# al-mcintyre/mCaller

Measured on NVIDIA B200. Metric: per-read site calls/sec, higher is better.
Workload: dtype f64

## Files before the change

### include/mcaller_b200.h

```cpp
#ifndef MCALLER_B200_H
#define MCALLER_B200_H

#include <stdint.h>

#ifdef __cplusplus
extern "C" {
#endif

#define MC_ABI_VERSION 3

#define MC_TILE_BYTES 3840
#define MC_TEXT_PAD 4096
#define MC_MAXK 8

enum {
    MC_OK = 0,
    MC_EINVAL = -1,
    MC_ECUDA = -2,
    MC_ECAPACITY = -3
};

typedef struct mc_refindex {
    int32_t n_contigs;
    int32_t k;
// ... 15 lines not shown
    uint16_t line_hi;
    uint16_t name_off;
    int32_t pos;
    int32_t event_idx;
    double diff;
    uint16_t name_len;
    uint16_t contig;
    uint8_t flags;
    uint8_t kbits_fwd;
    uint8_t kbits_rev;
    uint8_t pad;
} mc_record;

#define MC_RF_EQ 1u
#define MC_RF_CAND 2u
#define MC_RF_BADNUM 4u
#define MC_RF_BADIDX 8u
#define MC_RF_RAW 16u
#define MC_RF_NEWREAD 32u
#define MC_RF_SEGKNOWN 64u

enum {
    MC_C_LINES = 0,
    MC_C_KEPT,
    MC_C_RECORDS,
    MC_C_SHORT,
    MC_C_UNKNOWN_CONTIG,
    MC_C_NNN,
    MC_C_BADPOS,
    MC_C_LONGLINE,
    MC_C_OVERFLOW,
    MC_C_RUN_CURSOR,
    MC_C_QUIET,
    MC_C_COUNT = 16
};

typedef struct mc_call {
    int64_t read_off;
    double prob;
    double feat[MC_MAXK + 1];
    int32_t read_len;
    int32_t mpos;
    int32_t site;
    uint32_t close_rec;
    uint16_t win_contig;
    uint16_t chrom_contig;
    uint8_t kind;
    uint8_t rev;
    uint8_t n_empty;
    uint8_t empty_mask;
    uint8_t model_sel;
    uint8_t label;
    uint8_t err;
    uint8_t pad0;
    uint32_t seg;
    uint32_t pad1;
    uint32_t pad2;
} mc_call;

enum { MC_CALL = 0, MC_TOO_MANY_SKIPS = 1, MC_MULTI_M = 2, MC_NONE = 3  };
#define MC_CE_CONTEXT 1u
#define MC_CE_MODELKEY 2u
#define MC_CE_BADNUM 4u
#define MC_CE_COLUMN 8u
#define MC_CE_SPACING 16u

// ... 9 lines not shown
    const double *d_biases;
    int32_t n_trees;
    int32_t max_nodes;
    const int32_t *d_tree_off;
    const int32_t *d_left;
    const int32_t *d_right;
    const int32_t *d_feature;
    const double *d_threshold;
    const double *d_leaf_p1;
} mc_model;

typedef struct mc_qual_entry {
    uint64_t hash;
    uint32_t check;
    uint32_t len;
    double qual;
} mc_qual_entry;


int mc_version(void);
int mc_sizeof(int what);
const char *mc_last_error(void);

int mc_read_u64(const uint64_t *d_src, int64_t n, uint64_t *h_dst, void *stream);

int mc_scan(const uint8_t *d_text, int64_t nbytes, const mc_refindex *ref, int dense,
            mc_record *d_rec, int64_t rec_cap, uint32_t *d_tile_tab , uint32_t *d_run_tab ,
            uint64_t *d_counters, void *stream);

int mc_scan_run_len(int64_t nbytes);

int mc_scan_set_run_len(int run_len);

int64_t mc_num_tiles(int64_t nbytes);

int64_t mc_workspace_bytes(int64_t n);

int mc_order_records(const uint8_t *d_text, int64_t nbytes, const mc_refindex *ref, const uint32_t *d_tile_tab, int64_t n_tiles,
                     uint32_t *d_run_tab, int run_len, const mc_record *d_rec_in, int64_t rec_in_cap, const uint64_t *d_scan_counters,
                     mc_record *d_rec_out, int64_t rec_out_cap, uint64_t *d_n_out, uint32_t *d_seg_flags ,
                     uint32_t *d_run_first , void *d_ws, void *stream);

int mc_segment_reads(const uint8_t *d_text, mc_record *d_rec, const uint64_t *d_n_records, int64_t rec_cap,
                     uint32_t *d_seg_flags , const uint32_t *d_run_first, int64_t n_runs,
                     uint32_t *d_seg_start, uint64_t *d_nseg, void *d_ws, void *stream);

int mc_segment_quality(const uint8_t *d_text, const mc_record *d_rec, const uint32_t *d_seg_start, const uint64_t *d_nseg,
                       int64_t seg_cap, const mc_qual_entry *d_table, int64_t table_size, double *d_seg_qual, uint64_t *d_err,
                       void *stream);

int mc_build_windows(const mc_record *d_rec, const uint64_t *d_n_records, int64_t rec_cap, const uint32_t *d_seg_start,
                     const uint64_t *d_nseg, int64_t seg_cap, const double *d_seg_qual, const mc_refindex *ref, int skip_thresh,
                     double qual_thresh, int two_models, mc_call *d_calls, int64_t call_cap, uint32_t *d_seg_count,
                     uint64_t *d_ncalls, void *d_ws, double *d_spill, int64_t spill_cap, void *stream);

typedef struct mc_carry {
    mc_call row;
    uint32_t valid;
    int32_t first_kept_contig;
    uint64_t chunks;
    uint64_t pad[6];
} mc_carry;
int mc_carry_reset(mc_carry *d_carry, void *stream);
int mc_carry_rows(mc_call *d_rows, const uint64_t *d_ncalls, const mc_record *d_rec, const uint64_t *d_n_records,
                  const uint32_t *d_seg_start, const uint64_t *d_nseg, const double *d_seg_qual, double qual_thresh,
                  mc_carry *d_carry, uint64_t *d_nrows_out, const uint64_t *d_abort, void *stream);
// ... 103 lines not shown
```

### mcaller_b200/_lib.py

```python
import ctypes as C
import os

import numpy as np

HERE = os.path.dirname(os.path.abspath(__file__))
LIB_PATH = os.environ.get("MCALLER_B200_LIB") or os.path.join(HERE, "libmcaller_b200.so")

MC_TILE_BYTES = 3840
MC_TEXT_PAD = 4096
MC_MAXK = 8
MC_C_COUNT = 16
COUNTER_NAMES = ["lines", "kept", "records", "short", "unknown_contig", "nnn", "badpos", "longline", "overflow", "run_cursor", "quiet_chunks"]

MC_ABI_VERSION = 3
MC_CALL, MC_TOO_MANY_SKIPS, MC_MULTI_M, MC_NONE = 0, 1, 2, 3
MC_CE_CONTEXT, MC_CE_MODELKEY, MC_CE_BADNUM, MC_CE_COLUMN, MC_CE_SPACING = 1, 2, 4, 8, 16
MC_MLP, MC_LR, MC_GNB, MC_RF = 0, 1, 2, 3
PENDING = 0xFFFFFFFF


class RefIndex(C.Structure):
    _fields_ = [("n_contigs", C.c_int32), ("k", C.c_int32), ("d_names", C.c_void_p), ("d_name_off", C.c_void_p),
                ("d_base", C.c_void_p), ("d_len", C.c_void_p), ("d_site_fwd", C.c_void_p), ("d_site_rev", C.c_void_p),
                ("d_cand", C.c_void_p), ("d_rank_fwd", C.c_void_p), ("d_rank_rev", C.c_void_p), ("d_bases", C.c_void_p),
                ("total_bits", C.c_int64)]


class Model(C.Structure):
    _fields_ = [("kind", C.c_int32), ("n_in", C.c_int32), ("n_layers", C.c_int32), ("hidden_act", C.c_int32),
                ("sizes", C.c_int32 * 8), ("d_weights", C.c_void_p), ("d_biases", C.c_void_p), ("n_trees", C.c_int32),
                ("max_nodes", C.c_int32), ("d_tree_off", C.c_void_p), ("d_left", C.c_void_p), ("d_right", C.c_void_p),
                ("d_feature", C.c_void_p), ("d_threshold", C.c_void_p), ("d_leaf_p1", C.c_void_p)]


class SynthSpec(C.Structure):
    _fields_ = [("seed", C.c_uint64), ("n_contigs", C.c_int32), ("len_min", C.c_int32), ("len_max", C.c_int32),
                ("p_skip", C.c_int32), ("p_nnn", C.c_int32), ("margin", C.c_int32), ("meth", C.c_int32),
                ("d_names", C.c_void_p), ("d_name_off", C.c_void_p), ("d_contig_len", C.c_void_p),
                ("d_read_bounds", C.c_void_p), ("d_gbase", C.c_void_p), ("d_genome", C.c_void_p),
                ("d_meth_fwd", C.c_void_p), ("d_meth_rev", C.c_void_p), ("d_model_mean", C.c_void_p),
                ("d_model_sd", C.c_void_p)]


RECORD_DTYPE = np.dtype([("line_lo", "<u4"), ("line_hi", "<u2"), ("name_off", "<u2"), ("pos", "<i4"), ("event_idx", "<i4"),
                         ("diff", "<f8"), ("name_len", "<u2"), ("contig", "<u2"), ("flags", "u1"), ("kbits_fwd", "u1"), ("kbits_rev", "u1"), ("pad", "u1")])
# ... 12 lines not shown
class TrainJob(C.Structure):
    _fields_ = [("d_x", C.c_void_p), ("d_y", C.c_void_p), ("d_w", C.c_void_p), ("d_loss_curve", C.c_void_p), ("idx_off", C.c_int64),
                ("n", C.c_int32), ("d", C.c_int32), ("max_iter", C.c_int32), ("n_iter_no_change", C.c_int32), ("alpha", C.c_double),
                ("lr", C.c_double), ("tol", C.c_double), ("best_loss", C.c_double), ("n_iter", C.c_int32), ("no_improve", C.c_int32),
                ("stopped", C.c_int32), ("pad", C.c_int32)]


MC_TRAIN_HIDDEN, MC_TRAIN_BATCH = 100, 200

CARRY_BYTES = 192

QUAL_DTYPE = np.dtype([("hash", "<u8"), ("check", "<u4"), ("len", "<u4"), ("qual", "<f8")])
assert QUAL_DTYPE.itemsize == 24
DIFFS_ROW_DTYPE = np.dtype([("line_off", "<u8"), ("slot", "<u4"), ("values_off", "<u4"), ("values_len", "<u4"), ("prob_off", "<u4"),
                            ("prob_len", "<u4"), ("pad", "<u4")])
assert DIFFS_ROW_DTYPE.itemsize == 32


class McallerCudaError(RuntimeError):
    pass


_lib = None

_PROTOS = {
    "mc_version": (C.c_int, []),
    "mc_sizeof": (C.c_int, [C.c_int]),
    "mc_last_error": (C.c_char_p, []),
    "mc_read_u64": (C.c_int, [C.c_void_p, C.c_int64, C.c_void_p, C.c_void_p]),
    "mc_scan": (C.c_int, [C.c_void_p, C.c_int64, C.POINTER(RefIndex), C.c_int, C.c_void_p, C.c_int64, C.c_void_p, C.c_void_p, C.c_void_p,
                          C.c_void_p]),
    "mc_scan_run_len": (C.c_int, [C.c_int64]),
    "mc_scan_set_run_len": (C.c_int, [C.c_int]),
    "mc_num_tiles": (C.c_int64, [C.c_int64]),
    "mc_workspace_bytes": (C.c_int64, [C.c_int64]),
    "mc_order_records": (C.c_int, [C.c_void_p, C.c_int64, C.POINTER(RefIndex), C.c_void_p, C.c_int64, C.c_void_p, C.c_int, C.c_void_p,
                                   C.c_int64, C.c_void_p, C.c_void_p, C.c_int64, C.c_void_p, C.c_void_p, C.c_void_p, C.c_void_p, C.c_void_p]),
    "mc_segment_reads": (C.c_int, [C.c_void_p, C.c_void_p, C.c_void_p, C.c_int64, C.c_void_p, C.c_void_p, C.c_int64, C.c_void_p, C.c_void_p,
                                   C.c_void_p, C.c_void_p]),
    "mc_segment_quality": (C.c_int, [C.c_void_p, C.c_void_p, C.c_void_p, C.c_void_p, C.c_int64, C.c_void_p, C.c_int64, C.c_void_p,
                                     C.c_void_p, C.c_void_p]),
    "mc_build_windows": (C.c_int, [C.c_void_p, C.c_void_p, C.c_int64, C.c_void_p, C.c_void_p, C.c_int64, C.c_void_p, C.POINTER(RefIndex),
                                   C.c_int, C.c_double, C.c_int, C.c_void_p, C.c_int64, C.c_void_p, C.c_void_p, C.c_void_p, C.c_void_p,
                                   C.c_int64, C.c_void_p]),
    "mc_carry_reset": (C.c_int, [C.c_void_p, C.c_void_p]),
    "mc_carry_rows": (C.c_int, [C.c_void_p, C.c_void_p, C.c_void_p, C.c_void_p, C.c_void_p, C.c_void_p, C.c_void_p, C.c_double, C.c_void_p,
                                C.c_void_p, C.c_void_p, C.c_void_p]),
    "mc_chunk_guard": (C.c_int, [C.c_void_p, C.c_int64, C.c_void_p, C.c_int64, C.c_void_p, C.c_int64, C.c_void_p, C.c_int64, C.c_void_p,
                                 C.c_void_p, C.c_void_p]),
    "mc_carry_close": (C.c_int, [C.c_void_p, C.c_int, C.c_void_p, C.c_int, C.c_int, C.c_void_p, C.c_void_p, C.c_void_p, C.c_void_p,
                                 C.c_int64, C.c_void_p, C.c_void_p]),
    "mc_classify_workspace_bytes": (C.c_int64, [C.c_int64]),
    "mc_classify": (C.c_int, [C.c_void_p, C.c_void_p, C.c_int64, C.POINTER(Model), C.c_void_p, C.c_void_p]),
    "mc_hist_accumulate": (C.c_int, [C.c_void_p, C.c_void_p, C.c_int64, C.c_void_p, C.c_void_p, C.c_void_p, C.c_int64, C.c_void_p,
                                     C.c_void_p, C.c_int64, C.c_void_p, C.c_void_p, C.c_void_p]),
    "mc_count_calls": (C.c_int, [C.c_void_p, C.c_void_p, C.c_int64, C.c_void_p, C.c_void_p]),
    "mc_bed_select": (C.c_int, [C.c_void_p, C.c_void_p, C.c_int64, C.c_int64, C.c_double, C.c_int, C.c_void_p, C.c_void_p, C.c_void_p]),
    "mc_format_rows": (C.c_int64, [C.c_void_p, C.c_int64, C.c_void_p, C.c_void_p, C.c_int32, C.c_void_p, C.c_void_p, C.c_void_p, C.c_void_p,
                                   C.c_int32, C.c_int32, C.c_char_p, C.c_char_p, C.c_int32, C.c_int32, C.c_void_p, C.c_int64]),
    "mc_fastq_tiles": (C.c_int64, [C.c_int64]),
    "mc_fastq_index": (C.c_int, [C.c_void_p, C.c_int64, C.c_void_p, C.c_void_p, C.c_void_p, C.c_int64, C.c_void_p, C.c_void_p, C.c_void_p]),
    "mc_fastq_quality": (C.c_int, [C.c_void_p, C.c_int64, C.c_void_p, C.c_int64, C.c_void_p, C.c_int64, C.c_void_p, C.c_void_p, C.c_void_p,
                                   C.c_void_p]),
    "mc_synth_genome": (C.c_int, [C.POINTER(SynthSpec), C.c_void_p, C.c_int64, C.c_void_p]),
    "mc_synth_sizes": (C.c_int, [C.POINTER(SynthSpec), C.c_int64, C.c_int64, C.c_int64, C.c_void_p, C.c_void_p]),
    "mc_synth_write": (C.c_int, [C.POINTER(SynthSpec), C.c_int64, C.c_int64, C.c_int64, C.c_void_p, C.c_void_p, C.c_void_p]),
# ... 37 lines not shown
```

### mcaller_b200/csrc/scan.cu

```cuda
#include "parse.cuh"

namespace {

constexpr int CHUNK = MC_TILE_BYTES;
constexpr int LOOKB = 32;
constexpr int LOOKA = 224;
constexpr int WB = LOOKB + CHUNK + LOOKA;
constexpr int NW = WB / 32;
#ifndef MC_SCAN_WARPS
#define MC_SCAN_WARPS 24
#endif
#ifndef MC_SCAN_MIN_CTAS
#define MC_SCAN_MIN_CTAS 1
#endif
#ifndef MC_SCAN_RUN
#define MC_SCAN_RUN 128
#endif

constexpr int WARPS = MC_SCAN_WARPS;
constexpr int THREADS = WARPS * 32;
constexpr int LCAP = 32;
constexpr int RESERVE = 256;
static_assert(WB == 4096 && NW == 128, "chunk geometry");
static_assert(CHUNK % 16 == 0, "chunks must keep 16-byte alignment");
static_assert(MC_TEXT_PAD >= LOOKA + 64, "text padding must cover the look-ahead");

struct WarpSmem {
    alignas(16) uint8_t text[2][WB];
    alignas(16) uint32_t fs[NW + 8];
    alignas(16) uint32_t nl[NW + 4];
    uint16_t lstart[LCAP + 4];
    uint32_t cnt[8];
    unsigned long long key[4];
    alignas(8) unsigned long long bar[2];
    unsigned long long rname[8];
};

__device__ __forceinline__ uint32_t smem_u32(const void *p) { return (uint32_t)__cvta_generic_to_shared(p); }
__device__ __forceinline__ void mbar_init(unsigned long long *bar, uint32_t count) {
    asm volatile("mbarrier.init.shared::cta.b64 [%0], %1;" ::"r"(smem_u32(bar)), "r"(count) : "memory");
}
__device__ __forceinline__ void fence_barrier_init() { asm volatile("fence.mbarrier_init.release.cluster;" ::: "memory"); }
__device__ __forceinline__ void fence_proxy_async() { asm volatile("fence.proxy.async.shared::cta;" ::: "memory"); }
__device__ __forceinline__ void tma_load_1d(void *dst, const void *src, uint32_t bytes, unsigned long long *bar) {
    asm volatile("mbarrier.arrive.expect_tx.shared::cta.b64 _, [%0], %1;" ::"r"(smem_u32(bar)), "r"(bytes) : "memory");
    asm volatile("cp.async.bulk.shared::cluster.global.mbarrier::complete_tx::bytes [%0], [%1], %2, [%3];" ::"r"(smem_u32(dst)),
                 "l"(src), "r"(bytes), "r"(smem_u32(bar))
                 : "memory");
}
__device__ __forceinline__ bool mbar_wait(unsigned long long *bar, uint32_t parity) {
    const uint32_t a = smem_u32(bar);
    for (uint32_t spin = 0; spin < (1u << 26); ++spin) {
        uint32_t done;
        asm volatile(
            "{\n\t.reg .pred p;\n\t"
            "mbarrier.try_wait.parity.shared::cta.b64 p, [%1], %2;\n\t"
            "selp.u32 %0, 1, 0, p;\n\t}"
            : "=r"(done)
            : "r"(a), "r"(parity)
            : "memory");
        if (done) return true;
    }
    return false;
}

__device__ __forceinline__ uint32_t pack32(uint32_t m0, uint32_t m1, uint32_t m2, uint32_t m3, uint32_t m4, uint32_t m5,
                                           uint32_t m6, uint32_t m7) {
    const uint32_t lo = 0x08040201u, hi = 0x80402010u;
    const uint32_t a = __dp4a(m1, hi, __dp4a(m0, lo, 0u));
    const uint32_t b = __dp4a(m3, hi, __dp4a(m2, lo, 0u));
    const uint32_t c = __dp4a(m5, hi, __dp4a(m4, lo, 0u));
    const uint32_t d = __dp4a(m7, hi, __dp4a(m6, lo, 0u));
    return (a >> 7) + b * 2u + c * 512u + d * 131072u;
}

__device__ __noinline__ int select_fs_walk(const uint32_t *fs, int s, int n) {
    int w = s >> 5;
    uint32_t m = fs[w] & (0xFFFFFFFFu << (s & 31));
    int c = __popc(m);
    while (c <= n) {
        n -= c;
        if (++w >= NW) return NW * 32;
        m = fs[w];
        c = __popc(m);
    }
    for (; n > 0; --n) m &= m - 1u;
    return (w << 5) + __ffs(m) - 1;
}
__device__ __forceinline__ int next_bit(const uint32_t *m, int q) {
    int w = q >> 5;
    uint32_t v = m[w] & (0xFFFFFFFFu << (q & 31));
    while (v == 0u) {
        if (++w >= NW) return NW * 32;
        v = m[w];
    }
    return (w << 5) + __ffs(v) - 1;
}

template <bool WANT3>
__device__ __forceinline__ void line_fields(const WarpSmem &S, int s, int &f0, int &f1, int &f9, int &f11, int &f3) {
    const int w0 = s >> 5, sh = s & 31;
    const uint32_t a0 = S.fs[w0], a1 = S.fs[w0 + 1], a2 = S.fs[w0 + 2], a3 = S.fs[w0 + 3], a4 = S.fs[w0 + 4], a5 = S.fs[w0 + 5];
    const uint32_t W0 = __funnelshift_r(a0, a1, sh), W1 = __funnelshift_r(a1, a2, sh), W2 = __funnelshift_r(a2, a3, sh),
                   W3 = __funnelshift_r(a3, a4, sh), W4 = __funnelshift_r(a4, a5, sh);
    const int c0 = __popc(W0), c1 = c0 + __popc(W1), c2 = c1 + __popc(W2), c3 = c2 + __popc(W3), c4 = c3 + __popc(W4);
    if (c4 >= 12) {
        auto sel = [&](int k) {
            const int wi = (k >= c0) + (k >= c1) + (k >= c2) + (k >= c3);
            const uint32_t m = wi == 0 ? W0 : wi == 1 ? W1 : wi == 2 ? W2 : wi == 3 ? W3 : W4;
            const int base = wi == 0 ? 0 : wi == 1 ? c0 : wi == 2 ? c1 : wi == 3 ? c2 : c3;
            return s + 32 * wi + nth_bit(m, k - base);
        };
        if ((W0 & 1u) && c0 >= 2) {
            f0 = s;
            f1 = s + __ffs(W0 & (W0 - 1u)) - 1;
        } else {
            f0 = sel(0);
            f1 = sel(1);
        }
        if (WANT3) f3 = c0 >= 4 ? s + nth_bit(W0, 3) : sel(3);
        if (c2 <= 9 && c3 > 11) {
            uint32_t m = W3;
            const int j = 9 - c2;
#pragma unroll
            for (int t = 0; t < 4; ++t)
                if (j > t) m &= m - 1u;
            for (int t = 4; t < j; ++t) m &= m - 1u;
            f9 = s + 96 + __ffs(m) - 1;
            m &= m - 1u;
            m &= m - 1u;
            f11 = s + 96 + __ffs(m) - 1;
        } else {
            f9 = sel(9);
            f11 = sel(11);
        }
    } else {
        f0 = select_fs_walk(S.fs, s, 0);
        f1 = select_fs_walk(S.fs, s, 1);
        f9 = select_fs_walk(S.fs, s, 9);
        f11 = select_fs_walk(S.fs, s, 11);
        if (WANT3) f3 = select_fs_walk(S.fs, s, 3);
    }
}

__device__ __forceinline__ unsigned long long load8(const uint8_t *text, int q) {
    const uint32_t *wp = reinterpret_cast<const uint32_t *>(text + (q & ~3));
    const uint32_t w0 = wp[0], w1 = wp[1], w2 = wp[2];
    const int sh = 8 * (q & 3);
    const uint32_t lo = __funnelshift_r(w0, w1, sh), hi = __funnelshift_r(w1, w2, sh);
    return ((unsigned long long)hi << 32) | lo;
}

__device__ __forceinline__ int parse_pos8(unsigned long long k8, int &pos) {
    const uint32_t lo = (uint32_t)k8, hi = (uint32_t)(k8 >> 32);
    const uint32_t xl = lo ^ 0x30303030u, xh = hi ^ 0x30303030u;
    const uint32_t ndl = (((xl & 0x7f7f7f7fu) + 0x76767676u) | lo) & 0x80808080u;
    const uint32_t ndh = (((xh & 0x7f7f7f7fu) + 0x76767676u) | hi) & 0x80808080u;
    if ((ndl | ndh) == 0u) return -1;
    const int n = ndl ? ((__ffs(ndl) - 1) >> 3) : 4 + ((__ffs(ndh) - 1) >> 3);
    const uint32_t term = (n < 4 ? (lo >> (8 * n)) : (hi >> (8 * n - 32))) & 0xFFu;
    if (n == 0 || term > 0x20u) return 0;
    const int sh = 64 - 8 * n;
    const uint32_t H = sh < 32 ? __funnelshift_l(xl, xh, sh) : (xl << (sh - 32));
    const uint32_t L = sh < 32 ? (xl << sh) : 0u;
    pos = (int)(conv4(L) * 10000u + conv4(H));
    return 1;
}

__device__ __forceinline__ int token_len64(const uint8_t *text, int q) {
    for (int j = 0; j < 9; ++j) {
        const unsigned long long v = load8(text, q + 8 * j);
        const uint32_t lo = gt20_msb((uint32_t)v) ^ 0x80808080u, hi = gt20_msb((uint32_t)(v >> 32)) ^ 0x80808080u;
        if (lo) return 8 * j + ((__ffs(lo) - 1) >> 3);
        if (hi) return 8 * j + 4 + ((__ffs(hi) - 1) >> 3);
    }
    return -1;
}
__device__ __forceinline__ unsigned long long low_bytes(unsigned long long v, int n) {
    return n >= 8 ? v : (v & ((1ull << (8 * n)) - 1ull));
}
__device__ __forceinline__ bool token_is(const uint8_t *text, int q, int len, const unsigned long long *key) {
    bool eq = true;
    for (int j = 0; 8 * j < len; ++j) eq = eq && low_bytes(load8(text, q + 8 * j), len - 8 * j) == key[j];
    return eq;
}
__device__ __forceinline__ bool spans_equal(const uint8_t *text, int qa, int qb, int len) {
    bool eq = true;
    for (int j = 0; 8 * j < len; ++j) eq = eq && low_bytes(load8(text, qa + 8 * j) ^ load8(text, qb + 8 * j), len - 8 * j) == 0ull;
    return eq;
}
__device__ __forceinline__ int pos_digits8(unsigned long long k8) {
    const uint32_t lo = (uint32_t)k8, hi = (uint32_t)(k8 >> 32);
    const uint32_t xl = lo ^ 0x30303030u, xh = hi ^ 0x30303030u;
    const uint32_t ndl = (((xl & 0x7f7f7f7fu) + 0x76767676u) | lo) & 0x80808080u;
    const uint32_t ndh = (((xh & 0x7f7f7f7fu) + 0x76767676u) | hi) & 0x80808080u;
    return ndl ? ((__ffs(ndl) - 1) >> 3) : 4 + ((__ffs(ndh) - 1) >> 3);
}

enum { ST_KEPT = 1u, ST_CAND = 2u, ST_SHORT = 4u, ST_UNKNOWN = 8u, ST_NNN = 16u, ST_BADPOS = 32u };
// ... 5 lines not shown
    cid = known_cid >= 0 ? known_cid : contig_lookup(t, f0, R, hint);
    if (cid < 0) return ST_UNKNOWN;
    if (nnn_state > 0 || (nnn_state < 0 && is_nnnnnn(t, f9))) return ST_NNN;
    if (pos_state == 0 || (pos_state < 0 && !parse_uint(t, f1, pos))) return ST_BADPOS;
    uint32_t st = ST_KEPT;
    const int len = (cid == hint) ? hint_len : __ldg(R.d_len + cid);
    if (pos < len) {
        const int64_t g = ((cid == hint) ? hint_base : __ldg(R.d_base + cid)) + pos;
        if ((__ldg(R.d_cand + (g >> 5)) >> (g & 31)) & 1u) st |= ST_CAND;
    }
    return st;
}

__device__ __noinline__ uint32_t classify_from_global(const uint8_t *d_text, int64_t limit, int64_t goff, const mc_refindex &R, int hint,
                                                      int64_t hint_base, int hint_len, int &cid, int &pos) {
    const GlobalBytes t{d_text + goff, limit - goff};
    int nf = 0, f0 = 0, f1 = 0, f9 = 0;
    bool in_tok = false;
    for (int i = 0; i < (1 << 20); ++i) {
        const int c = t[i];
        if (c == 0x0a) break;
        const bool ws = c <= 0x20;
        if (!ws && !in_tok) {
            if (nf == 0) f0 = i; else if (nf == 1) f1 = i; else if (nf == 9) f9 = i;
            ++nf;
            in_tok = true;
            if (nf >= 12) break;
        } else if (ws) in_tok = false;
    }
    if (nf < 12) return ST_SHORT;
    return classify_line(t, f0, f1, f9, R, hint, hint_base, hint_len, -1, -1, -1, cid, pos);
}

template <bool RF>
__global__ void __launch_bounds__(THREADS, MC_SCAN_MIN_CTAS)
k_scan(const uint8_t *__restrict__ d_text, int64_t nbytes, int64_t text_limit16, int64_t n_chunks64, int run_len, mc_refindex R,
       int dense, mc_record *__restrict__ d_rec, unsigned long long rec_cap, uint32_t *__restrict__ d_tile_tab,
       uint32_t *__restrict__ d_run_tab, unsigned long long *__restrict__ d_counters) {
    extern __shared__ __align__(16) uint8_t smem_raw[];
    const int lane = threadIdx.x & 31, wib = threadIdx.x >> 5;
    WarpSmem &S = reinterpret_cast<WarpSmem *>(smem_raw)[wib];
    const int warp_global = (int)blockIdx.x * WARPS + wib;
    const int n_warps = (int)gridDim.x * WARPS;
    const int n_chunks = (int)n_chunks64;
    const int n_runs = (n_chunks + run_len - 1) / run_len;
    const uint32_t lt_mask = (1u << lane) - 1u;

    const uint32_t K7F = 0x7f7f7f7fu | ((uint32_t)((unsigned long long)nbytes >> 63) << 7);
    auto eq0a_r = [&](uint32_t w) -> uint32_t {
        const uint32_t t = ((w ^ 0x0a0a0a0au) & K7F) + K7F;
        return ~(t | w) & 0x80808080u;
    };

    int hint = -1;
    int64_t hint_base = 0;
    int hint_len = 0, hint_nlen = 0;
    unsigned long long hint_key = 0ull;
    auto set_hint = [&](int c) {
        hint = c;
        hint_base = __ldg(R.d_base + c);
        hint_len = __ldg(R.d_len + c);
        const int o0 = __ldg(R.d_name_off + c);
        hint_nlen = __ldg(R.d_name_off + c + 1) - o0;
        hint_key = 0ull;
        for (int j = 0; j < hint_nlen && j < 7; ++j) hint_key |= (unsigned long long)__ldg(R.d_names + o0 + j) << (8 * j);
        __syncwarp();
        if (lane < 4) {
            unsigned long long kk = 0ull;
            for (int j = 8 * lane; j < hint_nlen && j < 8 * lane + 8; ++j) kk |= (unsigned long long)__ldg(R.d_names + o0 + j) << (8 * (j & 7));
            S.key[lane] = kk;
        }
        __syncwarp();
    };
    set_hint(0);
    unsigned long long slot_cur = 0ull;
    unsigned slot_left = 0u;
    unsigned c_lines = 0, c_kept = 0;
    if (lane < 8) S.cnt[lane] = 0u;

    if (lane == 0) {
        mbar_init(&S.bar[0], 1);
        mbar_init(&S.bar[1], 1);
        fence_barrier_init();
    }
    __syncwarp();
    uint32_t phase0 = 0u, phase1 = 0u;

    const int64_t q_hi = text_limit16 - WB + LOOKB, q_tail = nbytes - WB + LOOKB;
    const int c_bulk_hi = q_hi < 0 ? -1 : (int)min(q_hi / CHUNK, (int64_t)0x7fffffff);
    const int c_tail_lo = q_tail < 0 ? 0 : (int)min(q_tail / CHUNK + 1, (int64_t)0x7fffffff);
    auto stage = [&](int c, int b) -> bool {
        const int64_t g0 = (int64_t)c * CHUNK - LOOKB;
        if (c >= 1 && c <= c_bulk_hi) {
            if (lane == 0) {
                fence_proxy_async();
                tma_load_1d(S.text[b], d_text + g0, WB, &S.bar[b]);
            }
            return true;
        }
        for (int i = lane; i < WB / 16; i += 32) {
            const int64_t g = g0 + 16 * i;
            uint4 v = make_uint4(0x0a0a0a0au, 0x0a0a0a0au, 0x0a0a0a0au, 0x0a0a0a0au);
            if (g >= 0 && g < text_limit16) v = __ldg(reinterpret_cast<const uint4 *>(d_text + g));
            *reinterpret_cast<uint4 *>(S.text[b] + 16 * i) = v;
        }
        return false;
    };

    int rname_len = -1;
    auto rf_all_match = [&](const uint8_t *text, int nm) -> bool {
        const int j = lane & 15;
// ... 190 lines not shown
        uint32_t filler = 0u;
        for (int pass0 = 0; pass0 < total_lines; pass0 += 32) {
            {
                int idx = my_first - pass0;
                uint32_t w0 = lsv.x, w1 = lsv.y, w2 = lsv.z, w3 = lsv.w;
                if (my_cnt <= 2) {
#pragma unroll
                    for (int t = 0; t < 2; ++t) {
                        if (t < my_cnt) {
                            const int jw = w0 ? 0 : w1 ? 1 : w2 ? 2 : 3;
                            const uint32_t m = w0 ? w0 : w1 ? w1 : w2 ? w2 : w3;
                            if (idx >= 0 && idx <= 32) S.lstart[idx] = (uint16_t)(32 * (4 * lane + jw) + __ffs(m) - 1);
                            ++idx;
                            const uint32_t cl = m & (m - 1u);
                            if (jw == 0) w0 = cl; else if (jw == 1) w1 = cl; else if (jw == 2) w2 = cl; else w3 = cl;
                        }
                    }
                } else {
                    const uint32_t wv[4] = {w0, w1, w2, w3};
#pragma unroll
                    for (int j = 0; j < 4; ++j) {
                        uint32_t m = wv[j];
                        while (m) {
                            const int b = __ffs(m) - 1;
                            m &= m - 1u;
                            if (idx >= 0 && idx <= 32) S.lstart[idx] = (uint16_t)(32 * (4 * lane + j) + b);
                            ++idx;
                        }
                    }
                }
            }
            __syncwarp();
            const int n_pass = min(32, total_lines - pass0);
            if (!full_ready) {
                full_ready = true;
                uint32_t prev_top = 0u;
#pragma unroll
                for (int r = 0; r < 4; ++r) {
                    const int w = 32 * r + lane;
                    const uint4 va = *reinterpret_cast<const uint4 *>(text + 32 * w);
                    const uint4 vb = *reinterpret_cast<const uint4 *>(text + 32 * w + 16);
                    const uint32_t nonws = pack32(gt20_msb(va.x), gt20_msb(va.y), gt20_msb(va.z), gt20_msb(va.w), gt20_msb(vb.x),
                                                  gt20_msb(vb.y), gt20_msb(vb.z), gt20_msb(vb.w));
                    const uint32_t top = nonws >> 31;
                    uint32_t pt = __shfl_up_sync(0xffffffffu, top, 1);
                    if (lane == 0) pt = prev_top;
                    prev_top = __shfl_sync(0xffffffffu, top, 31);
                    S.fs[w] = nonws & ~((nonws << 1) | pt);
                }
                if (lane < 8) S.fs[NW + lane] = 0u;
                if (!tail) {
                    constexpr int WLAST = (LOOKB + CHUNK - 1) >> 5, BLAST = (LOOKB + CHUNK - 1) & 31;
                    static_assert(NW - WLAST <= 32, "look-ahead words must fit one per lane");
                    int cand_e = NW * 32;
                    if (WLAST + lane < NW) {
                        uint32_t m = S.nl[WLAST + lane];
                        if (lane == 0) m &= 0xFFFFFFFFu << BLAST;
                        if (m) cand_e = 32 * (WLAST + lane) + __ffs(m) - 1;
                    }
                    e_last = __reduce_min_sync(0xffffffffu, cand_e);
                }
                __syncwarp();
            }
            uint32_t status = 0u;
            int cid = -1, pos = 0, s = 0;
            bool staged = false;
            int f3 = 0;
            if (lane < n_pass) {
                s = S.lstart[lane];
                const int e = (pass0 + lane + 1 < total_lines) ? (int)S.lstart[lane + 1] - 1 : (e_last >= 0 ? e_last : next_bit(S.nl, s));
                int f0, f1, f9, f11;
                line_fields<RF>(S, s, f0, f1, f9, f11, f3);
                if (f11 < e) {
                    staged = true;
                    const unsigned long long k8 = load8(text, f0);
                    const bool hit = hint_nlen <= 7 && (k8 & ((1ull << (8 * hint_nlen)) - 1ull)) == hint_key &&
                                     ((k8 >> (8 * hint_nlen)) & 0xFFull) <= 0x20ull;
                    int nnn = 0;
                    if (text[f9] == 'N') {
                        const unsigned long long m8 = load8(text, f9);
                        nnn = ((m8 & 0xFFFFFFFFFFFFull) == 0x4E4E4E4E4E4Eull && ((m8 >> 48) & 0xFFull) <= 0x20ull) ? 1 : 0;
                    }
                    const int pst = parse_pos8(load8(text, f1), pos);
                    status = classify_line(T, f0, f1, f9, R, hint, hint_base, hint_len, hit ? hint : -1, nnn, pst, cid, pos);
                } else if (e >= NW * 32 || f11 >= NW * 32) {
                    status = classify_from_global(d_text, nbytes + MC_TEXT_PAD - 64, G0 + s, R, hint, hint_base, hint_len, cid, pos);
                    atomicAdd(&S.cnt[4], 1u);
                } else {
                    status = ST_SHORT;
                }
            }
            if (status & (ST_SHORT | ST_UNKNOWN | ST_NNN | ST_BADPOS))
                atomicAdd(&S.cnt[(status & ST_SHORT) ? 0 : (status & ST_UNKNOWN) ? 1 : (status & ST_NNN) ? 2 : 3], 1u);

            const uint32_t kept_m = __ballot_sync(0xffffffffu, (status & ST_KEPT) != 0u);
            c_kept += (unsigned)__popc(kept_m);
            const uint32_t cand_m = __ballot_sync(0xffffffffu, (status & ST_CAND) != 0u);
            bool emit = false, filler_lane = false;
            if (RF) {
                const bool valid = lane < n_pass;
                const uint32_t unusual = __ballot_sync(0xffffffffu, valid && !staged);
                uint32_t new_m = 0u;
                if (unusual != 0u || rname_len < 1 || !rf_all_match(text, valid ? f3 : -1)) {
                int nq = 0, nlen = -1;
                if (valid && staged) {
                    nq = f3;
                    nlen = token_len64(text, nq);
                    if (nlen == 0) nlen = -1;
                }
                const int pq = __shfl_up_sync(0xffffffffu, nq, 1), plen = __shfl_up_sync(0xffffffffu, nlen, 1);
                bool same = false;
                if (valid && nlen > 0) {
                    if (lane == 0) same = nlen == rname_len && token_is(text, nq, nlen, S.rname);
                    else same = nlen == plen && spans_equal(text, nq, pq, nlen);
                }
                const uint32_t pass_m = n_pass >= 32 ? 0xFFFFFFFFu : ((1u << n_pass) - 1u);
                new_m = __ballot_sync(0xffffffffu, !same) & pass_m;
                const int lq = __shfl_sync(0xffffffffu, nq, n_pass - 1), llen = __shfl_sync(0xffffffffu, nlen, n_pass - 1);
                __syncwarp();
                if (llen > 0 && lane < 8) S.rname[lane] = 8 * lane < llen ? low_bytes(load8(text, lq + 8 * lane), llen - 8 * lane) : 0ull;
                rname_len = (llen > 0 && llen <= 63) ? llen : -1;
                __syncwarp();
                }
// ... 60 lines not shown
                slot_cur += ne;
                slot_left -= ne;
                n_emitted += ne;
            }
            __syncwarp();
        }
        if (lane == 0) {
            reinterpret_cast<uint2 *>(d_tile_tab)[chunk] =
                make_uint2((uint32_t)(slot_cur - n_emitted), n_emitted | (filler << 16) | ((uint32_t)(prev_state + 1) << 17));
        }
        run_total += n_emitted;
        run_filler |= filler;
        if (last_of_run) {
            if (lane == 0) reinterpret_cast<uint2 *>(d_run_tab)[chunk / run_len] = make_uint2(run_total, run_filler | ((uint32_t)(prev_state + 1) << 1));
            run_total = 0u;
            run_filler = 0u;
            prev_state = -1;
            rname_len = -1;
            read_has_kept = false;
        }
        chunk = next;
        run_end = next_end;
        buf ^= 1;
        cur_async = next_async;
    }

    __syncwarp();
    c_lines = __reduce_add_sync(0xffffffffu, c_lines);
    if (lane == 0) {
        if (c_lines) atomicAdd(&d_counters[MC_C_LINES], (unsigned long long)c_lines);
        if (c_kept) atomicAdd(&d_counters[MC_C_KEPT], (unsigned long long)c_kept);
        if (S.cnt[6]) atomicAdd(&d_counters[MC_C_QUIET], (unsigned long long)S.cnt[6]);
    }
    if (lane < 6) {
        const int which = lane == 0 ? MC_C_SHORT : lane == 1 ? MC_C_UNKNOWN_CONTIG : lane == 2 ? MC_C_NNN : lane == 3 ? MC_C_BADPOS
                        : lane == 4 ? MC_C_LONGLINE : MC_C_OVERFLOW;
        const unsigned v = S.cnt[lane];
        if (v) atomicAdd(&d_counters[which], (unsigned long long)v);
    }
}

}

static int g_run_len_override = 0;
extern "C" int mc_scan_set_run_len(int run_len) {
    const int before = g_run_len_override;
    g_run_len_override = run_len < 0 ? 0 : (run_len > 4096 ? 4096 : run_len);
    return before;
}

extern "C" int64_t mc_num_tiles(int64_t nbytes) { return nbytes <= 0 ? 0 : (nbytes + CHUNK - 1) / CHUNK; }

static int scan_geometry(int64_t n_chunks, int64_t *blocks_out, int *run_len_out) {
    int dev = 0, sms = 0;
    MC_CUDA_CHECK(cudaGetDevice(&dev));
    MC_CUDA_CHECK(cudaDeviceGetAttribute(&sms, cudaDevAttrMultiProcessorCount, dev));
    int64_t blocks = (n_chunks + WARPS - 1) / WARPS;
    const int64_t resident = (int64_t)sms * MC_SCAN_MIN_CTAS;
    if (blocks > resident) blocks = resident;
    int run_len = MC_SCAN_RUN;
    while (run_len > 1 && n_chunks < blocks * WARPS * 8 * (int64_t)run_len) run_len >>= 1;
    if (g_run_len_override > 0) run_len = g_run_len_override;
    *blocks_out = blocks;
    *run_len_out = run_len;
    return MC_OK;
}
extern "C" int mc_scan_run_len(int64_t nbytes) {
    const int64_t n_chunks = mc_num_tiles(nbytes);
    if (n_chunks == 0) return 1;
    int64_t blocks = 0;
    int run_len = 1;
    if (scan_geometry(n_chunks, &blocks, &run_len)) return -1;
    return run_len;
}

extern "C" int mc_scan(const uint8_t *d_text, int64_t nbytes, const mc_refindex *ref, int dense, mc_record *d_rec,
                       int64_t rec_cap, uint32_t *d_tile_tab, uint32_t *d_run_tab, uint64_t *d_counters, void *stream) {
    MC_REQUIRE(d_text && ref && d_rec && d_tile_tab && d_run_tab && d_counters, "null pointer");
    MC_REQUIRE(nbytes >= 0 && rec_cap >= 0, "negative size");
    MC_REQUIRE((reinterpret_cast<uintptr_t>(d_text) & 15) == 0, "d_text must be 16-byte aligned");
    MC_REQUIRE((reinterpret_cast<uintptr_t>(d_tile_tab) & 7) == 0, "d_tile_tab must be 8-byte aligned");
    MC_REQUIRE(ref->k >= 1 && ref->k <= MC_MAXK, "k out of range");
    MC_REQUIRE(ref->n_contigs >= 1 && ref->n_contigs < 65535, "contig count out of range");
    MC_REQUIRE(nbytes < (1ll << 47), "chunk too large");
    MC_REQUIRE(rec_cap < (1ll << 32), "record capacity must fit 32 bits");
    const int64_t n_chunks = mc_num_tiles(nbytes);
    if (n_chunks == 0) return MC_OK;
    MC_REQUIRE(n_chunks < (1ll << 30), "too many chunks (chunk of text larger than 4 TB)");
    const size_t smem = sizeof(WarpSmem) * WARPS;
    const bool read_first = dense == 2;
    MC_CUDA_CHECK(cudaFuncSetAttribute(read_first ? k_scan<true> : k_scan<false>, cudaFuncAttributeMaxDynamicSharedMemorySize, (int)smem));
    int64_t blocks = 0;
    int run_len = 1;
    {
        const int rc = scan_geometry(n_chunks, &blocks, &run_len);
        if (rc) return rc;
    }
    const int64_t text_limit16 = ((nbytes + MC_TEXT_PAD) / 16) * 16;
    MC_CUDA_CHECK(cudaMemsetAsync(d_counters + MC_C_RUN_CURSOR, 0, sizeof(uint64_t), (cudaStream_t)stream));
    if (read_first)
        k_scan<true><<<(unsigned)blocks, THREADS, smem, (cudaStream_t)stream>>>(d_text, nbytes, text_limit16, n_chunks, run_len, *ref, 0, d_rec,
                                                                               (unsigned long long)rec_cap, d_tile_tab, d_run_tab,
                                                                               reinterpret_cast<unsigned long long *>(d_counters));
    else
        k_scan<false><<<(unsigned)blocks, THREADS, smem, (cudaStream_t)stream>>>(d_text, nbytes, text_limit16, n_chunks, run_len, *ref, dense ? 1 : 0,
                                                                                d_rec, (unsigned long long)rec_cap, d_tile_tab, d_run_tab,
                                                                                reinterpret_cast<unsigned long long *>(d_counters));
    MC_LAUNCH_CHECK();
    return MC_OK;
}
```

Before: 48.96 million.

## Add fast settle path for scan lines matching the hinted contig

Adds a speculative fast path in the scan kernel. When every line in a pass matches the current contig hint name and parses a valid position, the warp builds field-start bits only for the words the needed lines touch, checks field counts and NNN only for candidate-relevant lines, and skips the full per-line classification. If any check fails, it falls back to the original path. Refactors the field selection into helpers, adds a legacy-parse toggle and diagnostic counters for how often the fast path is entered or rejected. The extra ballots and work are wasted on passes that fall back.

```diff
diff --git a/include/mcaller_b200.h b/include/mcaller_b200.h
--- a/include/mcaller_b200.h
+++ b/include/mcaller_b200.h
@@ -71,6 +71,11 @@
     MC_C_OVERFLOW,
     MC_C_RUN_CURSOR,
     MC_C_QUIET,
+    MC_C_NQ_CAND_ENTRY,
+    MC_C_NQ_RUN_FIRST,
+    MC_C_NQ_LOOK_CAND,
+    MC_C_NQ_LOOK_CONTIG,
+    MC_C_NQ_LOOK_POS,
     MC_C_COUNT = 16
 };
 
@@ -146,6 +151,8 @@
 
 int mc_scan_set_run_len(int run_len);
 
+int mc_scan_set_legacy_parse(int on);
+
 int64_t mc_num_tiles(int64_t nbytes);
 
 int64_t mc_workspace_bytes(int64_t n);
diff --git a/mcaller_b200/_lib.py b/mcaller_b200/_lib.py
--- a/mcaller_b200/_lib.py
+++ b/mcaller_b200/_lib.py
@@ -10,7 +10,8 @@
 MC_TEXT_PAD = 4096
 MC_MAXK = 8
 MC_C_COUNT = 16
-COUNTER_NAMES = ["lines", "kept", "records", "short", "unknown_contig", "nnn", "badpos", "longline", "overflow", "run_cursor", "quiet_chunks"]
+COUNTER_NAMES = ["lines", "kept", "records", "short", "unknown_contig", "nnn", "badpos", "longline", "overflow", "run_cursor", "quiet_chunks",
+                 "nq_cand_entry", "nq_run_first", "nq_look_cand", "nq_look_contig", "nq_look_pos"]
 
 MC_ABI_VERSION = 3
 MC_CALL, MC_TOO_MANY_SKIPS, MC_MULTI_M, MC_NONE = 0, 1, 2, 3
@@ -89,6 +90,7 @@
                           C.c_void_p]),
     "mc_scan_run_len": (C.c_int, [C.c_int64]),
     "mc_scan_set_run_len": (C.c_int, [C.c_int]),
+    "mc_scan_set_legacy_parse": (C.c_int, [C.c_int]),
     "mc_num_tiles": (C.c_int64, [C.c_int64]),
     "mc_workspace_bytes": (C.c_int64, [C.c_int64]),
     "mc_order_records": (C.c_int, [C.c_void_p, C.c_int64, C.POINTER(RefIndex), C.c_void_p, C.c_int64, C.c_void_p, C.c_int, C.c_void_p,
diff --git a/mcaller_b200/csrc/scan.cu b/mcaller_b200/csrc/scan.cu
--- a/mcaller_b200/csrc/scan.cu
+++ b/mcaller_b200/csrc/scan.cu
@@ -30,11 +30,12 @@
     alignas(16) uint32_t fs[NW + 8];
     alignas(16) uint32_t nl[NW + 4];
     uint16_t lstart[LCAP + 4];
-    uint32_t cnt[8];
+    uint32_t cnt[16];
     unsigned long long key[4];
     alignas(8) unsigned long long bar[2];
     unsigned long long rname[8];
 };
+static_assert(sizeof(WarpSmem) * WARPS <= 227 * 1024, "per-warp shared memory exceeds a block's limit");
 
 __device__ __forceinline__ uint32_t smem_u32(const void *p) { return (uint32_t)__cvta_generic_to_shared(p); }
 __device__ __forceinline__ void mbar_init(unsigned long long *bar, uint32_t count) {
@@ -97,43 +98,55 @@
     return (w << 5) + __ffs(v) - 1;
 }
 
+struct FsWindow {
+    uint32_t W0, W1, W2, W3, W4;
+    int c0, c1, c2, c3, c4;
+};
+__device__ __forceinline__ FsWindow fs_window(const WarpSmem &S, int s) {
+    const int w0 = s >> 5, sh = s & 31;
+    const uint32_t a0 = S.fs[w0], a1 = S.fs[w0 + 1], a2 = S.fs[w0 + 2], a3 = S.fs[w0 + 3], a4 = S.fs[w0 + 4], a5 = S.fs[w0 + 5];
+    FsWindow w;
+    w.W0 = __funnelshift_r(a0, a1, sh); w.W1 = __funnelshift_r(a1, a2, sh); w.W2 = __funnelshift_r(a2, a3, sh);
+    w.W3 = __funnelshift_r(a3, a4, sh); w.W4 = __funnelshift_r(a4, a5, sh);
+    w.c0 = __popc(w.W0); w.c1 = w.c0 + __popc(w.W1); w.c2 = w.c1 + __popc(w.W2); w.c3 = w.c2 + __popc(w.W3); w.c4 = w.c3 + __popc(w.W4);
+    return w;
+}
+__device__ __forceinline__ int fs_select(const FsWindow &w, int s, int k) {
+    const int wi = (k >= w.c0) + (k >= w.c1) + (k >= w.c2) + (k >= w.c3);
+    const uint32_t m = wi == 0 ? w.W0 : wi == 1 ? w.W1 : wi == 2 ? w.W2 : wi == 3 ? w.W3 : w.W4;
+    const int base = wi == 0 ? 0 : wi == 1 ? w.c0 : wi == 2 ? w.c1 : wi == 3 ? w.c2 : w.c3;
+    return s + 32 * wi + nth_bit(m, k - base);
+}
+__device__ __forceinline__ void fs_cols_10_12(const FsWindow &w, int s, int &f9, int &f11) {
+    if (w.c2 <= 9 && w.c3 > 11) {
+        uint32_t m = w.W3;
+        const int j = 9 - w.c2;
+#pragma unroll
+        for (int t = 0; t < 4; ++t)
+            if (j > t) m &= m - 1u;
+        for (int t = 4; t < j; ++t) m &= m - 1u;
+        f9 = s + 96 + __ffs(m) - 1;
+        m &= m - 1u;
+        m &= m - 1u;
+        f11 = s + 96 + __ffs(m) - 1;
+    } else {
+        f9 = fs_select(w, s, 9);
+        f11 = fs_select(w, s, 11);
+    }
+}
 template <bool WANT3>
 __device__ __forceinline__ void line_fields(const WarpSmem &S, int s, int &f0, int &f1, int &f9, int &f11, int &f3) {
-    const int w0 = s >> 5, sh = s & 31;
-    const uint32_t a0 = S.fs[w0], a1 = S.fs[w0 + 1], a2 = S.fs[w0 + 2], a3 = S.fs[w0 + 3], a4 = S.fs[w0 + 4], a5 = S.fs[w0 + 5];
-    const uint32_t W0 = __funnelshift_r(a0, a1, sh), W1 = __funnelshift_r(a1, a2, sh), W2 = __funnelshift_r(a2, a3, sh),
-                   W3 = __funnelshift_r(a3, a4, sh), W4 = __funnelshift_r(a4, a5, sh);
-    const int c0 = __popc(W0), c1 = c0 + __popc(W1), c2 = c1 + __popc(W2), c3 = c2 + __popc(W3), c4 = c3 + __popc(W4);
-    if (c4 >= 12) {
-        auto sel = [&](int k) {
-            const int wi = (k >= c0) + (k >= c1) + (k >= c2) + (k >= c3);
-            const uint32_t m = wi == 0 ? W0 : wi == 1 ? W1 : wi == 2 ? W2 : wi == 3 ? W3 : W4;
-            const int base = wi == 0 ? 0 : wi == 1 ? c0 : wi == 2 ? c1 : wi == 3 ? c2 : c3;
-            return s + 32 * wi + nth_bit(m, k - base);
-        };
-        if ((W0 & 1u) && c0 >= 2) {
+    const FsWindow w = fs_window(S, s);
+    if (w.c4 >= 12) {
+        if ((w.W0 & 1u) && w.c0 >= 2) {
             f0 = s;
-            f1 = s + __ffs(W0 & (W0 - 1u)) - 1;
+            f1 = s + __ffs(w.W0 & (w.W0 - 1u)) - 1;
         } else {
-            f0 = sel(0);
-            f1 = sel(1);
-        }
-        if (WANT3) f3 = c0 >= 4 ? s + nth_bit(W0, 3) : sel(3);
-        if (c2 <= 9 && c3 > 11) {
-            uint32_t m = W3;
-            const int j = 9 - c2;
-#pragma unroll
-            for (int t = 0; t < 4; ++t)
-                if (j > t) m &= m - 1u;
-            for (int t = 4; t < j; ++t) m &= m - 1u;
-            f9 = s + 96 + __ffs(m) - 1;
-            m &= m - 1u;
-            m &= m - 1u;
-            f11 = s + 96 + __ffs(m) - 1;
-        } else {
-            f9 = sel(9);
-            f11 = sel(11);
-        }
+            f0 = fs_select(w, s, 0);
+            f1 = fs_select(w, s, 1);
+        }
+        if (WANT3) f3 = w.c0 >= 4 ? s + nth_bit(w.W0, 3) : fs_select(w, s, 3);
+        fs_cols_10_12(w, s, f9, f11);
     } else {
         f0 = select_fs_walk(S.fs, s, 0);
         f1 = select_fs_walk(S.fs, s, 1);
@@ -165,6 +178,26 @@
     const uint32_t L = sh < 32 ? (xl << sh) : 0u;
     pos = (int)(conv4(L) * 10000u + conv4(H));
     return 1;
+}
+
+__device__ __forceinline__ int look_line(const uint8_t *text, int s0, const unsigned long long *key, int nlen, int64_t base, int len,
+                                         const uint32_t *d_cand) {
+    bool name_ok = true;
+    for (int j = 0; 8 * j <= nlen; ++j) {
+        const unsigned long long v = load8(text, s0 + 8 * j), kk = key[j];
+        const int rem = nlen - 8 * j;
+        if (rem >= 8) name_ok = name_ok && v == kk;
+        else name_ok = name_ok && (v & ((1ull << (8 * rem)) - 1ull)) == kk && ((v >> (8 * rem)) & 0xFFull) <= 0x20ull;
+    }
+    if (!name_ok) return -1;
+    int p = 0;
+    if (parse_pos8(load8(text, s0 + nlen + 1), p) != 1) return -2;
+    uint32_t cb = 0u;
+    if (p < len) {
+        const int64_t g = base + p;
+        cb = (__ldg(d_cand + (g >> 5)) >> (g & 31)) & 1u;
+    }
+    return (p << 1) | (int)cb;
 }
 
 __device__ __forceinline__ int token_len64(const uint8_t *text, int q) {
@@ -236,7 +269,7 @@
     return classify_line(t, f0, f1, f9, R, hint, hint_base, hint_len, -1, -1, -1, cid, pos);
 }
 
-template <bool RF>
+template <bool RF, bool LEGACY>
 __global__ void __launch_bounds__(THREADS, MC_SCAN_MIN_CTAS)
 k_scan(const uint8_t *__restrict__ d_text, int64_t nbytes, int64_t text_limit16, int64_t n_chunks64, int run_len, mc_refindex R,
        int dense, mc_record *__restrict__ d_rec, unsigned long long rec_cap, uint32_t *__restrict__ d_tile_tab,
@@ -249,6 +282,7 @@
     const int n_chunks = (int)n_chunks64;
     const int n_runs = (n_chunks + run_len - 1) / run_len;
     const uint32_t lt_mask = (1u << lane) - 1u;
+    constexpr bool SETTLE = !RF && !LEGACY;
 
     const uint32_t K7F = 0x7f7f7f7fu | ((uint32_t)((unsigned long long)nbytes >> 63) << 7);
     auto eq0a_r = [&](uint32_t w) -> uint32_t {
@@ -280,7 +314,7 @@
     unsigned long long slot_cur = 0ull;
     unsigned slot_left = 0u;
     unsigned c_lines = 0, c_kept = 0;
-    if (lane < 8) S.cnt[lane] = 0u;
+    if (lane < 16) S.cnt[lane] = 0u;
 
     if (lane == 0) {
         mbar_init(&S.bar[0], 1);
@@ -537,16 +571,98 @@
             }
             __syncwarp();
             const int n_pass = min(32, total_lines - pass0);
+            auto nonws_word = [&](int w) -> uint32_t {
+                const uint4 va = *reinterpret_cast<const uint4 *>(text + 32 * w);
+                const uint4 vb = *reinterpret_cast<const uint4 *>(text + 32 * w + 16);
+                return pack32(gt20_msb(va.x), gt20_msb(va.y), gt20_msb(va.z), gt20_msb(va.w), gt20_msb(vb.x), gt20_msb(vb.y),
+                              gt20_msb(vb.z), gt20_msb(vb.w));
+            };
+            auto find_e_last = [&]() -> int {
+                constexpr int WLAST = (LOOKB + CHUNK - 1) >> 5, BLAST = (LOOKB + CHUNK - 1) & 31;
+                static_assert(NW - WLAST <= 32, "look-ahead words must fit one per lane");
+                int cand_e = NW * 32;
+                if (WLAST + lane < NW) {
+                    uint32_t m = S.nl[WLAST + lane];
+                    if (lane == 0) m &= 0xFFFFFFFFu << BLAST;
+                    if (m) cand_e = 32 * (WLAST + lane) + __ffs(m) - 1;
+                }
+                return __reduce_min_sync(0xffffffffu, cand_e);
+            };
+            uint32_t status = 0u;
+            int cid = -1, pos = 0, s = 0;
+            bool staged = false;
+            int f3 = 0;
+
+            bool settled = false;
+            if (SETTLE && !dense && hint_nlen >= 1 && hint_nlen <= 31 && !tail && total_lines <= 32) {
+                int lv = 0;
+                if (lane < n_pass) {
+                    s = S.lstart[lane];
+                    lv = look_line(text, s, S.key, hint_nlen, hint_base, hint_len, R.d_cand);
+                }
+                const uint32_t other_m = __ballot_sync(0xffffffffu, lv == -1), badpos_m = __ballot_sync(0xffffffffu, lv == -2);
+                if (lane == 0) S.cnt[prev_state > 0 ? 7 : prev_state < 0 ? 8 : other_m ? 10 : badpos_m ? 11 : 9] += 1u;
+                if ((other_m | badpos_m) == 0u) {
+                    const uint32_t cm = __ballot_sync(0xffffffffu, lane < n_pass && (lv & 1));
+                    const uint32_t pass_m = n_pass >= 32 ? 0xFFFFFFFFu : ((1u << n_pass) - 1u);
+                    const uint32_t need_m = (cm | (cm << 1) | (prev_state != 0 ? 1u : 0u) | (1u << (n_pass - 1))) & pass_m;
+                    const bool need = (need_m >> lane) & 1u;
+                    uint32_t rounds = 0u;
+                    if (need) {
+                        const int lo = s >> 5, hi = min(lo + 5, NW - 1);
+                        rounds = (2u << (hi >> 5)) - (1u << (lo >> 5));
+                    }
+                    rounds = __reduce_or_sync(0xffffffffu, rounds);
+#pragma unroll
+                    for (int r = 0; r < 4; ++r) {
+                        if (rounds & (1u << r)) {
+                            const int w = 32 * r + lane;
+                            const uint32_t nonws = nonws_word(w);
+                            uint32_t pt = __shfl_up_sync(0xffffffffu, nonws >> 31, 1);
+                            if (lane == 0) pt = r ? (text[32 * w - 1] > 0x20 ? 1u : 0u) : 0u;
+                            S.fs[w] = nonws & ~((nonws << 1) | pt);
+                        }
+                    }
+                    if (lane < 8) S.fs[NW + lane] = 0u;
+                    const int e_end = find_e_last();
+                    __syncwarp();
+                    bool bad = false;
+                    if (need) {
+                        const int e = lane + 1 < n_pass ? (int)S.lstart[lane + 1] - 1 : e_end;
+                        const FsWindow fw = fs_window(S, s);
+                        bad = fw.c4 < 12;
+                        if (!bad) {
+                            int f9, f11;
+                            fs_cols_10_12(fw, s, f9, f11);
+                            bad = f11 >= e;
+                            if (text[f9] == 'N') {
+                                const unsigned long long m8 = load8(text, f9);
+                                bad = bad || ((m8 & 0xFFFFFFFFFFFFull) == 0x4E4E4E4E4E4Eull && ((m8 >> 48) & 0xFFull) <= 0x20ull);
+                            }
+                        }
+                        status = ST_KEPT | ((lv & 1) ? ST_CAND : 0u);
+                        cid = hint;
+                        pos = lv >> 1;
+                        staged = true;
+                    }
+                    settled = !__any_sync(0xffffffffu, bad);
+                    if (!settled) {
+                        status = 0u;
+                        cid = -1;
+                        pos = 0;
+                        staged = false;
+                    }
+                }
+            }
+
+            if (!settled) {
             if (!full_ready) {
                 full_ready = true;
                 uint32_t prev_top = 0u;
 #pragma unroll
                 for (int r = 0; r < 4; ++r) {
                     const int w = 32 * r + lane;
-                    const uint4 va = *reinterpret_cast<const uint4 *>(text + 32 * w);
-                    const uint4 vb = *reinterpret_cast<const uint4 *>(text + 32 * w + 16);
-                    const uint32_t nonws = pack32(gt20_msb(va.x), gt20_msb(va.y), gt20_msb(va.z), gt20_msb(va.w), gt20_msb(vb.x),
-                                                  gt20_msb(vb.y), gt20_msb(vb.z), gt20_msb(vb.w));
+                    const uint32_t nonws = nonws_word(w);
                     const uint32_t top = nonws >> 31;
                     uint32_t pt = __shfl_up_sync(0xffffffffu, top, 1);
                     if (lane == 0) pt = prev_top;
@@ -554,23 +670,9 @@
                     S.fs[w] = nonws & ~((nonws << 1) | pt);
                 }
                 if (lane < 8) S.fs[NW + lane] = 0u;
-                if (!tail) {
-                    constexpr int WLAST = (LOOKB + CHUNK - 1) >> 5, BLAST = (LOOKB + CHUNK - 1) & 31;
-                    static_assert(NW - WLAST <= 32, "look-ahead words must fit one per lane");
-                    int cand_e = NW * 32;
-                    if (WLAST + lane < NW) {
-                        uint32_t m = S.nl[WLAST + lane];
-                        if (lane == 0) m &= 0xFFFFFFFFu << BLAST;
-                        if (m) cand_e = 32 * (WLAST + lane) + __ffs(m) - 1;
-                    }
-                    e_last = __reduce_min_sync(0xffffffffu, cand_e);
-                }
+                if (!tail) e_last = find_e_last();
                 __syncwarp();
             }
-            uint32_t status = 0u;
-            int cid = -1, pos = 0, s = 0;
-            bool staged = false;
-            int f3 = 0;
             if (lane < n_pass) {
                 s = S.lstart[lane];
                 const int e = (pass0 + lane + 1 < total_lines) ? (int)S.lstart[lane + 1] - 1 : (e_last >= 0 ? e_last : next_bit(S.nl, s));
@@ -594,6 +696,7 @@
                 } else {
                     status = ST_SHORT;
                 }
+            }
             }
             if (status & (ST_SHORT | ST_UNKNOWN | ST_NNN | ST_BADPOS))
                 atomicAdd(&S.cnt[(status & ST_SHORT) ? 0 : (status & ST_UNKNOWN) ? 1 : (status & ST_NNN) ? 2 : 3], 1u);
@@ -720,9 +823,9 @@
         if (c_kept) atomicAdd(&d_counters[MC_C_KEPT], (unsigned long long)c_kept);
         if (S.cnt[6]) atomicAdd(&d_counters[MC_C_QUIET], (unsigned long long)S.cnt[6]);
     }
-    if (lane < 6) {
+    if (lane < 12 && lane != 6) {
         const int which = lane == 0 ? MC_C_SHORT : lane == 1 ? MC_C_UNKNOWN_CONTIG : lane == 2 ? MC_C_NNN : lane == 3 ? MC_C_BADPOS
-                        : lane == 4 ? MC_C_LONGLINE : MC_C_OVERFLOW;
+                        : lane == 4 ? MC_C_LONGLINE : lane == 5 ? MC_C_OVERFLOW : MC_C_NQ_CAND_ENTRY + (lane - 7);
         const unsigned v = S.cnt[lane];
         if (v) atomicAdd(&d_counters[which], (unsigned long long)v);
     }
@@ -731,6 +834,12 @@
 }
 
 static int g_run_len_override = 0;
+static int g_legacy_parse = 0;
+extern "C" int mc_scan_set_legacy_parse(int on) {
+    const int before = g_legacy_parse;
+    g_legacy_parse = on ? 1 : 0;
+    return before;
+}
 extern "C" int mc_scan_set_run_len(int run_len) {
     const int before = g_run_len_override;
     g_run_len_override = run_len < 0 ? 0 : (run_len > 4096 ? 4096 : run_len);
@@ -777,7 +886,8 @@
     MC_REQUIRE(n_chunks < (1ll << 30), "too many chunks (chunk of text larger than 4 TB)");
     const size_t smem = sizeof(WarpSmem) * WARPS;
     const bool read_first = dense == 2;
-    MC_CUDA_CHECK(cudaFuncSetAttribute(read_first ? k_scan<true> : k_scan<false>, cudaFuncAttributeMaxDynamicSharedMemorySize, (int)smem));
+    auto kern = read_first ? k_scan<true, false> : g_legacy_parse ? k_scan<false, true> : k_scan<false, false>;
+    MC_CUDA_CHECK(cudaFuncSetAttribute(kern, cudaFuncAttributeMaxDynamicSharedMemorySize, (int)smem));
     int64_t blocks = 0;
     int run_len = 1;
     {
@@ -786,14 +896,9 @@
     }
     const int64_t text_limit16 = ((nbytes + MC_TEXT_PAD) / 16) * 16;
     MC_CUDA_CHECK(cudaMemsetAsync(d_counters + MC_C_RUN_CURSOR, 0, sizeof(uint64_t), (cudaStream_t)stream));
-    if (read_first)
-        k_scan<true><<<(unsigned)blocks, THREADS, smem, (cudaStream_t)stream>>>(d_text, nbytes, text_limit16, n_chunks, run_len, *ref, 0, d_rec,
-                                                                               (unsigned long long)rec_cap, d_tile_tab, d_run_tab,
-                                                                               reinterpret_cast<unsigned long long *>(d_counters));
-    else
-        k_scan<false><<<(unsigned)blocks, THREADS, smem, (cudaStream_t)stream>>>(d_text, nbytes, text_limit16, n_chunks, run_len, *ref, dense ? 1 : 0,
-                                                                                d_rec, (unsigned long long)rec_cap, d_tile_tab, d_run_tab,
-                                                                                reinterpret_cast<unsigned long long *>(d_counters));
+    kern<<<(unsigned)blocks, THREADS, smem, (cudaStream_t)stream>>>(d_text, nbytes, text_limit16, n_chunks, run_len, *ref,
+                                                                  read_first ? 0 : (dense ? 1 : 0), d_rec, (unsigned long long)rec_cap,
+                                                                  d_tile_tab, d_run_tab, reinterpret_cast<unsigned long long *>(d_counters));
     MC_LAUNCH_CHECK();
     return MC_OK;
 }
```

Measured after the change: 46.45 million, median of 6. 5.1% lower.
